# xmed-lab/MOC

Measured on AMD Instinct MI355X. Metric: meta-steps/sec (train), slides/sec (eval) on 16-shot NSCLC synthetic bags, higher is better.
Workload: dtype f32; 1 GPU; NSCLC 2-way 16-shot train loop: 32 slides/epoch x 15000 patches x 512, topj 400, topk 10, row mask on; bag_storage=fp32, arithmetic=fp32 accumulate (MFMA), parallelism=single GPU, one Adam step per slide

## Files before the change

moc_amd/csrc/moc_meta_forward.hip:

```cpp
#include <cmath>
#include <cstddef>
#include <cstdlib>
#include "moc_meta_internal.h"

int moc_check_batch(const moc_batch_t* B, const char* who);

using namespace moc_meta_internal;

namespace {

struct FwdArgs {
    const unsigned char* X;
    const int64_t* row_off;
    const int64_t* sel_row;
    const int32_t* n_sel;
    const float* cand;
    const float *W1, *b1, *W2, *b2;
    const unsigned char* W1img;
    float *H1, *gates, *mixed;
    int64_t stride;
    int64_t base_host;
    int D, C, slide0;
    uint32_t use_bits;
    int cand_mode;
// ... 245 lines not shown
        const int r = threadIdx.x >> 2, i = threadIdx.x & 3;
        float z = 0.f;
        for (int h = 0; h < H; ++h) z = fmaf(Hs[r][h], W2s[i * H + h], z);
        z += b2_pre;
        const float g = 1.f / (1.f + expf(-z));
        Gs[r][i] = g;
        if (a.gates && row0 + r < S) a.gates[(base + row0 + r) * 4 + i] = g;
    }
    __syncthreads();
    for (int e = threadIdx.x; e < 16 * C; e += 256) {
        const int r = e & 15, c = e >> 4;
        if (row0 + r >= S) continue;
        float s0 = pre_c[0], s1 = pre_c[1], s2 = pre_c[2], s3 = pre_c[3];
        if (e >= 256) {
            const float* cd = cand_row(a, base, row0 + r);
            float m1, rden;
            cand_row_norm(a, cd, m1, rden);
            cand_class_scores(a, cd, c, m1, rden, s0, s1);
            cand_row_scores(a, cd, s2, s3);
        }
        float v = 0.f;
        if (a.use_bits & 1u) v = moc_fadd(v, moc_fmul(Gs[r][0], s0));
        if (a.use_bits & 2u) v = moc_fadd(v, moc_fmul(Gs[r][1], s1));
        if (a.use_bits & 4u) v = moc_fadd(v, moc_fmul(Gs[r][2], s2));
        if (a.use_bits & 8u) v = moc_fadd(v, moc_fmul(Gs[r][3], s3));
        a.mixed[(int64_t)c * a.stride + base + row0 + r] = v;
    }
    if (TILES && a.tile_on && threadIdx.x < 16 * C) {
        const int r = threadIdx.x & 15, c = threadIdx.x >> 4;
        const bool ok = row0 + r < S;
        float v = 0.f;
        if (a.use_bits & 1u) v = moc_fadd(v, moc_fmul(Gs[r][0], pre_c[0]));
        if (a.use_bits & 2u) v = moc_fadd(v, moc_fmul(Gs[r][1], pre_c[1]));
        if (a.use_bits & 4u) v = moc_fadd(v, moc_fmul(Gs[r][2], pre_c[2]));
        if (a.use_bits & 8u) v = moc_fadd(v, moc_fmul(Gs[r][3], pre_c[3]));
        const float4 lam4 = {Gs[r][0], Gs[r][1], Gs[r][2], Gs[r][3]};
        const float4 sc4 = {pre_c[0], pre_c[1], pre_c[2], pre_c[3]};
        tile_emit(a.tile, fr.tile_slot0 / TILE_R + (int64_t)c * fr.tile_cap + blockIdx.x, ok, v, row0 + r, rid_e, lam4, sc4);
    }
    MOC_STAMP(2);
}

constexpr int FKS_PSTR = H + 4;
__host__ __device__ constexpr int fks_lds_bytes(int D) {
    return 3 * 16 * D * 2 + 4 * 16 * FKS_PSTR * 4 + 16 * (H + 1) * 4 + 16 * 4 * 4 + 4 * H * 4;
}
template <int DQ, bool STATS>
__global__ __launch_bounds__(1024) void meta_forward_ksplit_kernel(FwdArgs a) {
    extern __shared__ __attribute__((aligned(16))) unsigned char smem[];
    constexpr int D = DQ * 256;
    uint4* xt = reinterpret_cast<uint4*>(smem);
    float* part = reinterpret_cast<float*>(smem + (size_t)3 * 16 * D * 2);
    float (*Hs)[H + 1] = reinterpret_cast<float (*)[H + 1]>(part + 4 * 16 * FKS_PSTR);
    float (*Gs)[4] = reinterpret_cast<float (*)[4]>(reinterpret_cast<float*>(Hs) + 16 * (H + 1));
    float* W2s = reinterpret_cast<float*>(Gs) + 16 * 4;
    const FwdRun fr = fwd_run_setup(a);
    const int b = fr.b;
    const int64_t base = fr.base;
    const int S = fr.S >= 0 ? fr.S : a.n_sel[b];
    const int row0 = blockIdx.x * 16;
    if (row0 >= S) return;
    const int t = threadIdx.x, lane = t & 63;
    const int wave = __builtin_amdgcn_readfirstlane(t >> 6);
    const int ht = wave & 3, kq = wave >> 2;
    MOC_STAMP(0);
    MOC_STAMP_MIN(31);
    MOC_STAMP_MAX(32);
    constexpr int64_t row_bytes = (int64_t)D * 4;
    constexpr int cpl = DQ;
    const int sr = min(row0 + wave, S - 1);
    const int64_t rid = a.sel_row[base + sr];
    const unsigned char* rp = a.X + rid * row_bytes + lane * 16;
    MOC_STAMP_DRAIN(3);
    constexpr int QK = D / 128;
    const uint4* wi = reinterpret_cast<const uint4*>(fr.W1img) + ((size_t)ht * (D / 32) + (size_t)kq * QK) * 3 * 64 + lane + (rid >> 63);
    uint4 xv[cpl];
#pragma unroll
    for (int i = 0; i < cpl; ++i) xv[i] = *reinterpret_cast<const uint4*>(rp + i * 1024);
    uint4 wv[QK * 3];
#pragma unroll
    for (int q = 0; q < QK * 3; ++q) wv[q] = wi[q * 64];
    constexpr int cpr = D / 8;
    uint2* xt2 = reinterpret_cast<uint2*>(smem);
#pragma unroll
    for (int i = 0; i < cpl; ++i) {
        uint2 tv[3];
        fwd_split4(xv[i], tv);
        const int o = (wave * cpr + (((lane + i * 64) >> 1) ^ wave)) * 2 + (lane & 1);
#pragma unroll
        for (int p = 0; p < 3; ++p) xt2[p * 16 * cpr * 2 + o] = tv[p];
    }
    MOC_STAMP(5);
    __syncthreads();
    MOC_STAMP(6);
    const int C = a.C;
    float pre_c[4] = {0.f, 0.f, 0.f, 0.f};
    const int er = t & 15, ec = t >> 4;
    const bool e_ok = ec < C && row0 + er < S;
    if constexpr (STATS) {
        if (e_ok) {
            const float* cd = cand_row(a, base, row0 + er);
            float m1, rden;
            cand_row_norm(a, cd, m1, rden);
            cand_class_scores(a, cd, ec, m1, rden, pre_c[0], pre_c[1]);
            cand_row_scores(a, cd, pre_c[2], pre_c[3]);
        }
    } else {
        const float* cd = a.cand + base + min(row0 + er, S - 1);
        const int cc = ec < C ? ec : C - 1;
        pre_c[0] = cd[(int64_t)cc * a.stride];
        pre_c[1] = cd[(int64_t)(C + cc) * a.stride];
        pre_c[2] = cd[(int64_t)(2 * C) * a.stride];
        pre_c[3] = cd[(int64_t)(2 * C + 1) * a.stride];
    }
    const float w2_pre = fr.W2[t & 255];
    const float bias = fr.b1[t & 63];
    const float b2_pre = fr.b2[t & 3];
    int64_t rid_e = 0;
    if (a.tile_on) rid_e = a.sel_row[base + min(row0 + er, S - 1)];
    __builtin_amdgcn_sched_barrier(0);
    f32x4_t acc = {0.f, 0.f, 0.f, 0.f};
    {
        const int r = lane & 15;
        const uint4* xr = xt + r * cpr;
        const int c0 = kq * QK * 4 + (lane >> 4);
#pragma unroll
        for (int kk = 0; kk < QK; ++kk) {
            const int c = (c0 + kk * 4) ^ r;
            const uint4 xa[3] = {xr[c], xr[16 * cpr + c], xr[32 * cpr + c]};
            acc = fwd_mfma6(xa, wv[kk * 3], wv[kk * 3 + 1], wv[kk * 3 + 2], acc);
        }
    }
#ifdef MOC_STAMPS
    asm volatile("v_add_f32 %0, %0, 0" : "+v"(acc[0]));
#endif
    MOC_STAMP(1);
    {
        float* pp = part + (size_t)(kq * 16 + (lane >> 4) * 4) * FKS_PSTR + ht * 16 + (lane & 15);
#pragma unroll
        for (int i = 0; i < 4; ++i) pp[i * FKS_PSTR] = acc[i];
        if (t < 4 * H) W2s[t] = w2_pre;
    }
    __syncthreads();
    MOC_STAMP(7);
    {
        const int r = t >> 6, h = t & 63;
        const float* pp = part + (size_t)r * FKS_PSTR + h;
        const float pre = moc_fadd(moc_fadd(moc_fadd(pp[0], pp[16 * FKS_PSTR]), pp[32 * FKS_PSTR]), pp[48 * FKS_PSTR]);
        const float hv = fmaxf(moc_fadd(pre, bias), 0.f);
        Hs[r][h] = hv;
        if (a.H1 && row0 + r < S) a.H1[(base + row0 + r) * H + h] = hv;
    }
    __syncthreads();
    MOC_STAMP(8);
    if (t < 64) {
        const int r = t >> 2, i = t & 3;
        float z = 0.f;
        for (int h = 0; h < H; ++h) z = fmaf(Hs[r][h], W2s[i * H + h], z);
        z += b2_pre;
        const float g = 1.f / (1.f + expf(-z));
        Gs[r][i] = g;
        if (a.gates && row0 + r < S) a.gates[(base + row0 + r) * 4 + i] = g;
    }
    __syncthreads();
    MOC_STAMP(9);
    if (ec < C) {
        float v = 0.f;
        if (a.use_bits & 1u) v = moc_fadd(v, moc_fmul(Gs[er][0], pre_c[0]));
        if (a.use_bits & 2u) v = moc_fadd(v, moc_fmul(Gs[er][1], pre_c[1]));
        if (a.use_bits & 4u) v = moc_fadd(v, moc_fmul(Gs[er][2], pre_c[2]));
        if (a.use_bits & 8u) v = moc_fadd(v, moc_fmul(Gs[er][3], pre_c[3]));
        if (e_ok) a.mixed[(int64_t)ec * a.stride + base + row0 + er] = v;
        if (a.tile_on) {
            const float4 lam4 = {Gs[er][0], Gs[er][1], Gs[er][2], Gs[er][3]};
            const float4 sc4 = {pre_c[0], pre_c[1], pre_c[2], pre_c[3]};
            tile_emit(a.tile, fr.tile_slot0 / TILE_R + (int64_t)ec * fr.tile_cap + blockIdx.x, e_ok, v, row0 + er, rid_e, lam4, sc4);
        }
    }
    MOC_STAMP(2);
    MOC_STAMP_MAX(30);
}

template <bool F16>
__global__ __launch_bounds__(256) void meta_forward64_kernel(FwdArgs a) {
    __shared__ __attribute__((aligned(16))) uint4 xt[64 * 32];
    __shared__ float Hs[64][H + 1];
    __shared__ float Gs[64][4];
    __shared__ float W2s[4 * H];
    const int b = a.slide0 + blockIdx.y;
    const int64_t base = a.row_off[b];
    const int S = a.n_sel[b];
    const int row0 = blockIdx.x * 64;
    if (row0 >= S) return;
    const int lane = threadIdx.x & 63, wave = threadIdx.x >> 6;
    const int C = a.C;
    const int er = threadIdx.x & 63, ec0 = threadIdx.x >> 6;
    const bool erow_ok = row0 + er < S;
    const float* ecd = cand_row(a, base, erow_ok ? row0 + er : row0);
    float es2 = 0.f, es3 = 0.f, em1 = 0.f, erd = 0.f, es0[8], es1[8];
    if (erow_ok) {
        cand_row_scores(a, ecd, es2, es3);
        cand_row_norm(a, ecd, em1, erd);
    }
#pragma unroll
    for (int it = 0; it < 8; ++it) {
        const int c = ec0 + 4 * it;
        es0[it] = es1[it] = 0.f;
        if (erow_ok && c < C) cand_class_scores(a, ecd, c, em1, erd, es0[it], es1[it]);
    }
    const float w2_pre = a.W2[threadIdx.x & 255];
    const float bias = a.b1[wave * 16 + (lane & 15)];
    const float b2_pre = a.b2[threadIdx.x & 3];
    const int64_t row_bytes = (int64_t)a.D * 2;
    const int U = (int)(row_bytes / 512), KST = (int)(row_bytes / 64);
    const unsigned char* rp[8];
#pragma unroll
    for (int j = 0; j < 8; ++j) {
        const int sr = min(row0 + wave * 16 + 2 * j + (lane >> 5), S - 1);
        rp[j] = a.X + a.sel_row[base + sr] * row_bytes + (lane & 31) * 16;
    }
    f32x4_t acc[4];
#pragma unroll
    for (int rt = 0; rt < 4; ++rt) acc[rt] = f32x4_t{0.f, 0.f, 0.f, 0.f};
    for (int u = 0; u < U; ++u) {
        if (u > 0) __syncthreads();
        uint4 xv[8];
#pragma unroll
        for (int j = 0; j < 8; ++j) xv[j] = *reinterpret_cast<const uint4*>(rp[j] + (int64_t)u * 512);
        uint4 wv[8 * 3];
        const uint4* wi = reinterpret_cast<const uint4*>(a.W1img) + ((size_t)wave * KST + (size_t)u * 8) * 3 * 64 + lane;
#pragma unroll
        for (int q = 0; q < 8 * 3; ++q) wv[q] = wi[q * 64];
#pragma unroll
        for (int j = 0; j < 8; ++j) {
            const int r = wave * 16 + 2 * j + (lane >> 5);
            xt[r * 32 + ((lane & 31) ^ (r & 15))] = xv[j];
        }
        __syncthreads();
#pragma unroll
        for (int kk = 0; kk < 8; ++kk) {
#pragma unroll
            for (int rt = 0; rt < 4; ++rt) {
                const int r = rt * 16 + (lane & 15);
                const uint4 A = xt[r * 32 + ((kk * 4 + (lane >> 4)) ^ (r & 15))];
#pragma unroll
                for (int t = 0; t < 3; ++t) acc[rt] = moc_mfma_half<F16>(A, wv[kk * 3 + t], acc[rt]);
            }
        }
    }
    {
        const int hcol = wave * 16 + (lane & 15);
#pragma unroll
        for (int rt = 0; rt < 4; ++rt)
#pragma unroll
            for (int i = 0; i < 4; ++i) {
                const float pre = F16 ? acc[rt][i] * (1.f / MOC_F16_W1_SCALE) : acc[rt][i];
                Hs[rt * 16 + (lane >> 4) * 4 + i][hcol] = fmaxf(moc_fadd(pre, bias), 0.f);
            }
        W2s[threadIdx.x] = w2_pre;
    }
    __syncthreads();
    if (a.H1) {
        for (int e = threadIdx.x; e < 64 * H; e += 256) {
            const int r = e >> 6, h = e & 63;
            if (row0 + r < S) a.H1[(base + row0 + r) * H + h] = Hs[r][h];
        }
    }
    {
        const int r = threadIdx.x >> 2, i = threadIdx.x & 3;
        float z = 0.f;
        for (int h = 0; h < H; ++h) z = fmaf(Hs[r][h], W2s[i * H + h], z);
        z += b2_pre;
        const float g = 1.f / (1.f + expf(-z));
        Gs[r][i] = g;
        if (a.gates && row0 + r < S) a.gates[(base + row0 + r) * 4 + i] = g;
    }
    __syncthreads();
    for (int cb = 0; cb < C; cb += 32) {
        if (cb > 0) {
#pragma unroll
            for (int it = 0; it < 8; ++it) {
                const int c = cb + ec0 + 4 * it;
                if (erow_ok && c < C) cand_class_scores(a, ecd, c, em1, erd, es0[it], es1[it]);
            }
        }
#pragma unroll
        for (int it = 0; it < 8; ++it) {
            const int c = cb + ec0 + 4 * it;
            if (!erow_ok || c >= C) continue;
            float v = 0.f;
            if (a.use_bits & 1u) v = moc_fadd(v, moc_fmul(Gs[er][0], es0[it]));
            if (a.use_bits & 2u) v = moc_fadd(v, moc_fmul(Gs[er][1], es1[it]));
            if (a.use_bits & 4u) v = moc_fadd(v, moc_fmul(Gs[er][2], es2));
            if (a.use_bits & 8u) v = moc_fadd(v, moc_fmul(Gs[er][3], es3));
            a.mixed[(int64_t)c * a.stride + base + row0 + er] = v;
        }
    }
}

constexpr int F128_ROWS = 128;
constexpr int f128_kc(int st) { return st == 2 ? 2 : 1; }
constexpr int f128_wgs(int st) { return st == 2 ? 3 : 4; }
constexpr int f128_buf(int kc) { return (F128_ROWS / 16) * kc * 1024; }
constexpr int f128_xb(int kc) { return 2 * f128_buf(kc) > F128_ROWS * (H + 1) * 4 ? 2 * f128_buf(kc) : F128_ROWS * (H + 1) * 4; }
constexpr int f128_lds(int kc) { return f128_xb(kc) + F128_ROWS * 4 * 4 + 4 * H * 4; }
typedef unsigned __attribute__((ext_vector_type(4))) fu32x4_t;
template <int OFF>
__device__ __forceinline__ void fwd_lds16(fu32x4_t& dst, unsigned addr) {
    asm volatile("ds_read_b128 %0, %1 offset:%2" : "=&v"(dst) : "v"(addr), "n"(OFF) : "memory");
}
__device__ __forceinline__ void fwd_touch4(fu32x4_t (&v)[4]) {
    asm volatile("" : "+v"(v[0]), "+v"(v[1]), "+v"(v[2]), "+v"(v[3]));
}

constexpr int F128_MODELS = 4;
constexpr int F128_ENSEMBLE = 8;
constexpr int F128_BY_SLIDE = 16;
constexpr int F128_ENS_MAX_C = 64;
constexpr int f128_bound(int stm) { return (stm & F128_ENSEMBLE) ? f128_wgs(stm & 3) - 1 : f128_wgs(stm & 3); }
template <int STM, bool DENSE = false>
__global__ __launch_bounds__(256, f128_bound(STM)) void meta_forward128_kernel(FwdArgs a) {
    constexpr int ST = STM & 3;
    constexpr bool MODELS = (STM & F128_MODELS) != 0;
    constexpr bool ENS = (STM & F128_ENSEMBLE) != 0;
    constexpr bool BYS = (STM & F128_BY_SLIDE) != 0;
    static_assert(!ENS || (MODELS && DENSE), "the ensemble mode is a dense models mode");
    static_assert(!BYS || (!MODELS && !DENSE), "a model per slide: the union rows, one model each");
    constexpr int F128_KC = f128_kc(ST), F128_BUF = f128_buf(F128_KC), F128_XB = f128_xb(F128_KC);
    constexpr bool F16 = ST == 1;
    constexpr int WPC = 3 * (ST == 2 ? F128_KC / 2 : F128_KC);
    constexpr int ESZ = ST == 2 ? 4 : 2;
    extern __shared__ __attribute__((aligned(16))) unsigned char smem[];
    float (*Hs)[H + 1] = reinterpret_cast<float (*)[H + 1]>(smem);
    float (*Gs)[4] = reinterpret_cast<float (*)[4]>(smem + F128_XB);
    float* W2s = reinterpret_cast<float*>(smem + F128_XB + F128_ROWS * 4 * 4);
    const int b = a.slide0 + blockIdx.y;
    const int64_t base = a.row_off[b];
    const int S = DENSE ? (int)(a.row_off[b + 1] - base) : a.n_sel[b];
    const int row0 = blockIdx.x * F128_ROWS;
    if (row0 >= S) return;
    const int lane = threadIdx.x & 63, wave = threadIdx.x >> 6;
    const int C = a.C;
#ifdef MOC_FWD_DIAG
    const unsigned diag = a.use_bits >> 8;
#else
    constexpr unsigned diag = 0;
#endif
    const int er = threadIdx.x & 127, ec0 = threadIdx.x >> 7;
    const bool erow_ok = row0 + er < S;
    const float* ecd = DENSE ? a.stats + base + (erow_ok ? row0 + er : row0) : cand_row(a, base, erow_ok ? row0 + er : row0);
    float es2 = 0.f, es3 = 0.f, em1 = 0.f, erd = 0.f, es0[8];
    if (erow_ok) {
        cand_row_scores(a, ecd, es2, es3);
        cand_row_norm(a, ecd, em1, erd);
    }
#pragma unroll
    for (int it = 0; it < 8; ++it) {
        const int c = ec0 + 2 * it;
        es0[it] = 0.f;
        if (erow_ok && c < C) es0[it] = ecd[(int64_t)c * a.stride];
    }
    float w2_pre = a.W2[threadIdx.x & 255];
    float bias = a.b1[wave * 16 + (lane & 15)];
    float b2_pre = a.b2[threadIdx.x & 3];
    int bys_m = 0;
    if constexpr (BYS) {
        bys_m = min(max(a.model_of_slide[b], 0), a.n_runs - 1);
        const int64_t po = (int64_t)bys_m * a.par_stride;
        w2_pre = a.W2[po + (threadIdx.x & 255)];
        bias = a.b1[po + wave * 16 + (lane & 15)];
        b2_pre = a.b2[po + (threadIdx.x & 3)];
    }
    const int64_t row_bytes = (int64_t)a.D * ESZ;
    const int KK = (int)(row_bytes / 64), nchunk = KK / F128_KC;
    const unsigned char* rp[2];
    int64_t xbase = 0;
    if constexpr (DENSE) xbase = a.x_off ? a.x_off[b] : base;
#pragma unroll
    for (int j = 0; j < 2; ++j) {
        const int sr = min(row0 + (wave * 2 + j) * 16 + (lane & 15), S - 1);
        rp[j] = a.X + (DENSE ? xbase + sr : a.sel_row[base + sr]) * row_bytes + (lane >> 4) * 16;
    }
    typedef const __attribute__((address_space(1))) void* gptr_t;
    typedef __attribute__((address_space(3))) void* lptr_t;
    auto issue_x = [&](int c, int buf) {
        unsigned char* dst = smem + buf * F128_BUF;
#pragma unroll
        for (int j = 0; j < 2; ++j)
#pragma unroll
            for (int kl = 0; kl < F128_KC; ++kl)
                __builtin_amdgcn_global_load_lds((gptr_t)(rp[j] + ((int64_t)c * F128_KC + kl) * 64),
                                                 (lptr_t)(dst + ((wave * 2 + j) * F128_KC + kl) * 1024), 16, 0, 0);
    };
    int m = 0;
next_model:
    if (MODELS && m > 0) {
        const int64_t po = (int64_t)m * a.par_stride;
        const float *W2m = a.W2, *b1m = a.b1, *b2m = a.b2;
        if constexpr (ENS) asm volatile("" : "+s"(W2m), "+s"(b1m), "+s"(b2m));
        w2_pre = W2m[po + (threadIdx.x & 255)];
        bias = b1m[po + wave * 16 + (lane & 15)];
        b2_pre = b2m[po + (threadIdx.x & 3)];
    }
    int64_t cstride = a.stride;
    if constexpr (ENS) {
        asm volatile("" : "+s"(cstride), "+v"(rp[0]), "+v"(rp[1]), "+v"(ecd));
    }
    const unsigned char* w1img = MODELS ? a.W1img + (int64_t)m * a.img_stride : a.W1img;
    if constexpr (BYS) w1img += (int64_t)bys_m * a.img_stride;
    float* mixed = MODELS ? a.mixed + (int64_t)m * C * a.stride : a.mixed;
    const fu32x4_t* wimg = reinterpret_cast<const fu32x4_t*>(w1img) + (size_t)wave * (a.D / 32) * 3 * 64 + lane;
    auto load_w = [&](int c, fu32x4_t (&wv)[WPC]) {
#pragma unroll
        for (int q = 0; q < WPC; ++q) wv[q] = wimg[((size_t)c * WPC + q) * 64];
    };
    f32x4_t acc[8];
#pragma unroll
    for (int r = 0; r < 8; ++r) acc[r] = f32x4_t{0.f, 0.f, 0.f, 0.f};
    f32x4_t tot[ST == 2 ? 8 : 1] = {};
    const int qchunks = nchunk / 4;
    const unsigned lds0 = (unsigned)(uintptr_t)smem + lane * 16;
    const unsigned lds0f = (unsigned)(uintptr_t)smem + (lane >> 5) * 1024 + ((((lane >> 4) & 1) * 32) + (lane & 15)) * 16;
    auto body = [&](int c, const fu32x4_t (&cur)[WPC], fu32x4_t (&nxt)[WPC]) {
        if (c + 1 < nchunk) {
            if (!(diag & 2u)) load_w(c + 1, nxt);
            if (!(diag & 4u)) issue_x(c + 1, (c + 1) & 1);
        }
        if constexpr (ST == 2) {
            const unsigned buf = lds0f + (c & 1) * F128_BUF;
#pragma unroll
            for (int rt = 0; rt < 8; ++rt) {
                fu32x4_t P[2];
                fwd_lds16<0>(P[0], buf + rt * F128_KC * 1024);
                fwd_lds16<256>(P[1], buf + rt * F128_KC * 1024);
                asm volatile("s_waitcnt lgkmcnt(0)" ::: "memory");
                asm volatile("" : "+v"(P[0]), "+v"(P[1]));
                if (!(diag & 1u)) {
                    uint4 xa[3];
                    fwd_split8(__builtin_bit_cast(uint4, P[0]), __builtin_bit_cast(uint4, P[1]), xa);
                    acc[rt] = fwd_mfma6(xa, cur[0], cur[1], cur[2], acc[rt]);
                }
            }
            if ((c + 1) % qchunks == 0) {
                const bool first = c + 1 == qchunks;
#pragma unroll
                for (int r = 0; r < 8; ++r) fwd_fold_quarter(tot[r], acc[r], first);
            }
            __syncthreads();
            return;
        }
        const unsigned buf = lds0 + (c & 1) * F128_BUF;
        fu32x4_t A0[2], A1[2];
#pragma unroll
        for (int r = 0; r < 2; ++r) fwd_lds16<0>(A0[r], buf + (r * F128_KC + 0) * 1024);
#pragma unroll
        for (int st = 0; st < F128_KC * 4; ++st) {
            const int kl = st >> 2, g = st & 3;
            fu32x4_t (&Ac)[2] = (st & 1) ? A1 : A0;
            fu32x4_t (&An)[2] = (st & 1) ? A0 : A1;
            if (st + 1 < F128_KC * 4) {
                const int kl_n = (st + 1) >> 2, g_n = (st + 1) & 3;
#pragma unroll
                for (int r = 0; r < 2; ++r) fwd_lds16<0>(An[r], buf + ((g_n * 2 + r) * F128_KC + kl_n) * 1024);
                asm volatile("s_waitcnt lgkmcnt(2)" ::: "memory");
            } else {
                asm volatile("s_waitcnt lgkmcnt(0)" ::: "memory");
            }
            asm volatile("" : "+v"(Ac[0]), "+v"(Ac[1]));
            if (!(diag & 1u)) {
#pragma unroll
                for (int r = 0; r < 2; ++r)
#pragma unroll
                    for (int t = 0; t < 3; ++t) acc[g * 2 + r] = moc_mfma_half<F16>(Ac[r], cur[kl * 3 + t], acc[g * 2 + r]);
            }
        }
        __syncthreads();
    };
    fu32x4_t wA[WPC], wB[WPC];
    load_w(0, wA);
    issue_x(0, 0);
    __syncthreads();
    for (int c = 0; c < nchunk; c += 2) {
        body(c, wA, wB);
        if (c + 1 < nchunk) body(c + 1, wB, wA);
    }
    {
        const int hcol = wave * 16 + (lane & 15);
        if constexpr (ST == 2) {
#pragma unroll
            for (int r = 0; r < 8; ++r) acc[r] = tot[r];
        }
#pragma unroll
        for (int r = 0; r < 8; ++r)
#pragma unroll
            for (int i = 0; i < 4; ++i) {
                const float pre = F16 ? acc[r][i] * (1.f / MOC_F16_W1_SCALE) : acc[r][i];
                Hs[r * 16 + (lane >> 4) * 4 + i][hcol] = fmaxf(moc_fadd(pre, bias), 0.f);
            }
        W2s[threadIdx.x] = w2_pre;
    }
    __syncthreads();
    if (!ENS && a.H1) {
        for (int e = threadIdx.x; e < F128_ROWS * H; e += 256) {
            const int r = e >> 6, h = e & 63;
            if (row0 + r < S) a.H1[(base + row0 + r) * H + h] = Hs[r][h];
        }
    }
#pragma unroll
    for (int rr = 0; rr < 2; ++rr) {
        const int r = (threadIdx.x >> 2) + rr * 64, i = threadIdx.x & 3;
        float z = 0.f;
        for (int h = 0; h < H; ++h) z = fmaf(Hs[r][h], W2s[i * H + h], z);
        z += b2_pre;
        const float g = 1.f / (1.f + expf(-z));
        Gs[r][i] = g;
        if constexpr (ENS) {
            float* gts = a.gates;
            asm volatile("" : "+s"(gts));
            if (gts && row0 + r < S) {
                float* gp = gts + (base + row0 + r) * 4 + i;
                const float sg = m > 0 ? *gp + g : g;
                *gp = m + 1 == a.n_runs ? sg / (float)a.n_runs : sg;
            }
        } else {
            if (a.gates && row0 + r < S) a.gates[(base + row0 + r) * 4 + i] = g;
        }
    }
    __syncthreads();
    float* Ms = reinterpret_cast<float*>(smem);
    if (erow_ok && !(diag & 8u)) {
        const float g0 = Gs[er][0], g1 = Gs[er][1], g2 = Gs[er][2], g3 = Gs[er][3];
        for (int cb = 0; cb < C; cb += 16) {
            if (cb > 0 || (MODELS && m > 0 && C > 16)) {
#pragma unroll
                for (int it = 0; it < 8; ++it) {
                    const int c = cb + ec0 + 2 * it;
                    if (c < C) es0[it] = ecd[(int64_t)c * cstride];
                }
            }
            float es1[8];
#pragma unroll
            for (int it = 0; it < 8; ++it) {
                const int c = cb + ec0 + 2 * it;
                es1[it] = 0.f;
                if (c < C) es1[it] = a.cand_mode == 2 ? moc_softmax_from(es0[it], em1, erd) : ecd[(int64_t)(C + c) * cstride];
            }
#pragma unroll
            for (int it = 0; it < 8; ++it) {
                const int c = cb + ec0 + 2 * it;
                if (c >= C) continue;
                const float s1 = es1[it];
                float v = 0.f;
                if (a.use_bits & 1u) v = moc_fadd(v, moc_fmul(g0, es0[it]));
                if (a.use_bits & 2u) v = moc_fadd(v, moc_fmul(g1, s1));
                if (a.use_bits & 4u) v = moc_fadd(v, moc_fmul(g2, es2));
                if (a.use_bits & 8u) v = moc_fadd(v, moc_fmul(g3, es3));
                if constexpr (ENS) Ms[er * C + c] = v;
                else mixed[(int64_t)c * cstride + base + row0 + er] = v;
            }
        }
    }
    if constexpr (ENS) {
        __syncthreads();
        if (erow_ok) {
            const float* mr = Ms + er * C;
            const float scale = a.ens_scale;
            float mx = -INFINITY, se = 0.f;
            for (int c = 0; c < C; ++c) mx = fmaxf(mx, scale * mr[c]);
            for (int c = 0; c < C; ++c) se += expf(scale * mr[c] - mx);
            float* __restrict__ pmean = a.mixed + base + row0 + er;
            float* __restrict__ pm2 = a.H1 ? a.H1 + base + row0 + er : nullptr;
            const bool last = m + 1 == a.n_runs;
            const float kf = (float)(m + 1);
            for (int cb = 0; cb < C; cb += 16) {
                float mu[8], m2[8];
#pragma unroll
                for (int it = 0; it < 8; ++it) {
                    const int c = cb + ec0 + 2 * it;
                    mu[it] = 0.f;
                    m2[it] = 0.f;
                    if (m > 0 && c < C) {
                        mu[it] = pmean[(int64_t)c * cstride];
                        if (pm2) m2[it] = pm2[(int64_t)c * cstride];
                    }
                }
#pragma unroll
                for (int it = 0; it < 8; ++it) {
                    const int c = cb + ec0 + 2 * it;
                    if (c >= C) continue;
                    const float p = expf(scale * mr[c] - mx) / se;
                    const float d = p - mu[it];
                    const float mu1 = m > 0 ? mu[it] + d / kf : p;
                    const float m21 = m > 0 ? m2[it] + d * (p - mu1) : 0.f;
                    pmean[(int64_t)c * cstride] = mu1;
                    if (pm2) pm2[(int64_t)c * cstride] = last ? sqrtf(m21 / (float)a.n_runs) : m21;
                }
            }
        }
        __syncthreads();
    }
    if constexpr (MODELS) {
        if (++m < a.n_runs) goto next_model;
    }
}

__global__ __launch_bounds__(256) void fixed_mix_kernel(FwdArgs a, int mode) {
    const int b = a.slide0 + blockIdx.y;
    const int64_t base = a.row_off[b];
    const int S = a.n_sel[b], C = a.C;
    const int s = blockIdx.x * 256 + threadIdx.x;
    if (s >= S) return;
    const float* cd = a.cand + base + s;
    const float s2 = cd[(int64_t)(2 * C) * a.stride], s3 = cd[(int64_t)(2 * C + 1) * a.stride];
    for (int c = 0; c < C; ++c) {
        const float s0 = cd[(int64_t)c * a.stride], s1 = cd[(int64_t)(C + c) * a.stride];
        float v;
        if (mode == 0) v = moc_fadd(moc_fadd(moc_fadd(moc_fmul(0.25f, s0), moc_fmul(0.25f, s1)), moc_fmul(0.25f, s2)), moc_fmul(0.25f, s3));
        else if (mode == 1) v = moc_fadd(moc_fadd(moc_fadd(s0, s1), s2), s3);
        else v = fmaxf(fmaxf(s0, s1), fmaxf(s2, s3));
        a.mixed[(int64_t)c * a.stride + base + s] = v;
    }
}

}

namespace moc_meta_internal {

int check_meta(const moc_batch_t* B, const moc_meta_t* M, const moc_meta_ws_t* ws, const char* who,
               bool need_adam, bool need_grad, bool need_h1) {
    MOC_REQUIRE(M && ws, "%s: null meta/ws", who);
    MOC_REQUIRE(M->H == H, "%s: hidden width %d unsupported (must be %d)", who, M->H, H);
    MOC_REQUIRE(M->D == B->D, "%s: meta D=%d != batch D=%d", who, M->D, B->D);
    MOC_REQUIRE(M->W1 && M->b1 && M->W2 && M->b2, "%s: null parameter", who);
    MOC_REQUIRE((!need_h1 || (ws->H1 && ws->gates)) && ws->mixed && ws->pooled && ws->topk_idx && ws->topk_cnt && ws->loss && ws->pred,
                "%s: null work array", who);
    MOC_REQUIRE(B->sel_row && B->n_sel && B->cand, "%s: batch has no phase-A outputs", who);
    MOC_REQUIRE(!(B->flags & MOC_CAND_FROM_STATS) || !(need_adam || need_grad),
                "%s: a MOC_CAND_FROM_STATS batch has no materialised candidate scores (evaluation only)", who);
    MOC_REQUIRE(B->topk <= 256 && B->C <= 256, "%s: topk/C too large for the fused step (<= 256)", who);
    if (need_adam)
        MOC_REQUIRE(M->m_W1 && M->m_b1 && M->m_W2 && M->m_b2 && M->v_W1 && M->v_b1 && M->v_W2 && M->v_b2,
                    "%s: null Adam state", who);
    if (need_grad) MOC_REQUIRE(M->g_W1 && M->g_b1 && M->g_W2 && M->g_b2, "%s: null gradient output", who);
    if (need_adam || need_grad) MOC_REQUIRE(ws->pair_dh && ws->pair_row && ws->n_pair, "%s: null backward scratch", who);
    return MOC_OK;
}

int launch_w1_images(const moc_batch_t* B, const moc_meta_t* M, const moc_runs_t* R, hipStream_t s) {
    MOC_REQUIRE(M->W1_image, "meta: W1_image buffer is null (moc_w1_image_bytes)");
    w1_image_kernel<<<dim3(H * B->D / 256, R ? R->n_runs : 1), 256, 0, s>>>(M->W1, B->D, (unsigned char*)M->W1_image, B->dtype,
                                                                            R ? R->par_stride : 0, R ? R->image_stride : 0);
    MOC_CHECK_LAUNCH(R ? "moc_w1_image(runs)" : "moc_w1_image");
    return MOC_OK;
}

int s_bound(const moc_batch_t* B) {
    const int64_t by_sel = (int64_t)B->topj * (2 * B->C + 2);
    return (int)(by_sel < B->max_rows ? by_sel : B->max_rows);
}

}

namespace {

constexpr int F64_SINGLE_ROWS = 16384;

FwdArgs fwd_args(const moc_batch_t* B, const moc_meta_t* M, int slide0, uint32_t use_bits) {
    FwdArgs a = {};
    a.X = (const unsigned char*)B->X; a.row_off = B->row_off; a.sel_row = B->sel_row; a.n_sel = B->n_sel;
    a.cand = B->cand; a.W1 = M->W1; a.b1 = M->b1; a.W2 = M->W2; a.b2 = M->b2;
    a.W1img = (const unsigned char*)M->W1_image;
    a.stride = B->total_rows;
    a.D = B->D; a.C = B->C; a.slide0 = slide0; a.use_bits = use_bits;
    a.base_host = -1;
    a.S_host = -1;
    if (B->flags & MOC_CAND_FROM_STATS) {
        a.cand_mode = (B->flags & MOC_STATS_COMPACT) ? 2 : 1;
        a.stats = B->stats; a.sel_idx = B->sel_idx;
    }
    return a;
}

template <int MODE, bool DENSE>
int launch_f128(const FwdArgs& a, dim3 grid, int dtype, hipStream_t s, const char* who) {
    static std::once_flag attr;
    std::call_once(attr, [] {
        (void)hipFuncSetAttribute((const void*)meta_forward128_kernel<MODE + 0, DENSE>, hipFuncAttributeMaxDynamicSharedMemorySize, f128_lds(f128_kc(0)));
        (void)hipFuncSetAttribute((const void*)meta_forward128_kernel<MODE + 1, DENSE>, hipFuncAttributeMaxDynamicSharedMemorySize, f128_lds(f128_kc(1)));
        (void)hipFuncSetAttribute((const void*)meta_forward128_kernel<MODE + 2, DENSE>, hipFuncAttributeMaxDynamicSharedMemorySize, f128_lds(f128_kc(2)));
    });
    if (dtype == MOC_F16) meta_forward128_kernel<MODE + 1, DENSE><<<grid, 256, f128_lds(f128_kc(1)), s>>>(a);
    else if (dtype == MOC_BF16) meta_forward128_kernel<MODE + 0, DENSE><<<grid, 256, f128_lds(f128_kc(0)), s>>>(a);
    else meta_forward128_kernel<MODE + 2, DENSE><<<grid, 256, f128_lds(f128_kc(2)), s>>>(a);
    MOC_CHECK_LAUNCH(who);
    return MOC_OK;
}

int launch_ksplit(const FwdArgs& a, dim3 grid, hipStream_t s, const char* who) {
    static std::once_flag attr;
    std::call_once(attr, [] {
#define MOC_KS_ATTR(DQ)                                                                                                                                  \
    (void)hipFuncSetAttribute((const void*)meta_forward_ksplit_kernel<DQ, false>, hipFuncAttributeMaxDynamicSharedMemorySize, fks_lds_bytes(DQ * 256)); \
    (void)hipFuncSetAttribute((const void*)meta_forward_ksplit_kernel<DQ, true>, hipFuncAttributeMaxDynamicSharedMemorySize, fks_lds_bytes(DQ * 256))
        MOC_KS_ATTR(2); MOC_KS_ATTR(3); MOC_KS_ATTR(4);
#undef MOC_KS_ATTR
    });
    const int lds = fks_lds_bytes(a.D);
#define MOC_KS_LAUNCH(DQ)                                                                        \
    do {                                                                                         \
        if (a.cand_mode) meta_forward_ksplit_kernel<DQ, true><<<grid, 1024, lds, s>>>(a);         \
        else meta_forward_ksplit_kernel<DQ, false><<<grid, 1024, lds, s>>>(a);                    \
    } while (0)
    switch (a.D / 256) {
        case 1: MOC_KS_LAUNCH(1); break;
        case 2: MOC_KS_LAUNCH(2); break;
        case 3: MOC_KS_LAUNCH(3); break;
        default: MOC_KS_LAUNCH(4); break;
    }
#undef MOC_KS_LAUNCH
    MOC_CHECK_LAUNCH(who);
    return MOC_OK;
}

int64_t dense_rows(const moc_batch_t* B, int slide0, int n) {
    if (!B->row_off_host) return B->max_rows;
    int64_t rows = 0;
    for (int q = slide0; q < slide0 + n; ++q) {
        const int64_t nq = B->row_off_host[q + 1] - B->row_off_host[q];
        rows = nq > rows ? nq : rows;
    }
    return rows;
}

}

int moc_meta_internal::launch_forward(const moc_batch_t* B, const moc_meta_t* M, const moc_meta_ws_t* ws, int slide0, int n,
                                      uint32_t use_bits, hipStream_t s, bool emit_tiles, const moc_runs_t* runs, int64_t w2_stride) {
    MOC_REQUIRE(!(B->flags & MOC_CAND_FROM_STATS) || (B->stats && B->sel_idx),
                "moc_meta_forward: MOC_CAND_FROM_STATS needs the batch's stats and sel_idx");
    FwdArgs a = fwd_args(B, M, slide0, use_bits);
#ifdef MOC_FWD_DIAG
    if (const char* dg = getenv("MOC_FWD_DIAG")) a.use_bits |= (uint32_t)atoi(dg) << 8;
#endif
    a.H1 = ws->H1; a.gates = ws->gates; a.mixed = ws->mixed;
    if (n == 1 && B->row_off_host) a.base_host = B->row_off_host[slide0];
    if (emit_tiles) {
        MOC_REQUIRE(n == 1 && B->row_off_host && ws->tile_ws, "moc_meta_forward: tile records need one slide, row_off_host and ws->tile_ws");
        a.tile_on = 1;
        a.tile = tile_carve(ws->tile_ws, tile_slots(B->total_rows, B->n_slides, B->C));
        a.tile_cap = moc_cdiv(B->row_off_host[slide0 + 1] - a.base_host, 16);
        a.tile_slot0 = ((a.base_host >> 4) + slide0) * (int64_t)B->C * TILE_R;
    }
    dim3 grid(moc_cdiv(s_bound(B), 16), n);
    const bool s_known = n == 1 && B->n_sel_host != nullptr;
    if (s_known && !runs) {
        a.S_host = B->n_sel_host[slide0];
        MOC_REQUIRE(a.S_host >= 0 && a.S_host <= s_bound(B), "moc_meta_forward: n_sel_host[%d] = %d is not a row count of this batch (bound %d)",
                    slide0, a.S_host, s_bound(B));
        grid.x = a.S_host > 0 ? moc_cdiv(a.S_host, 16) : 1;
    }
    if (runs) {
        MOC_REQUIRE(n == 1 && a.tile_on, "moc_train_steps_runs: the batched forward needs the tile-record step");
        a.n_runs = runs->n_runs; a.slide_stride = runs->slide_stride;
        a.par_stride = runs->par_stride; a.img_stride = runs->image_stride; a.w2_stride = w2_stride;
        int s_max = 0;
        for (int r = 0; r < runs->n_runs; ++r) {
            const int sl = slide0 + r * runs->slide_stride;
            a.base_r[r] = B->row_off_host[sl];
            a.tile_cap_r[r] = moc_cdiv(B->row_off_host[sl + 1] - B->row_off_host[sl], 16);
            a.tile_slot0_r[r] = ((B->row_off_host[sl] >> 4) + sl) * (int64_t)B->C * TILE_R;
            if (s_known) {
                a.S_r[r] = B->n_sel_host[sl];
                MOC_REQUIRE(a.S_r[r] >= 0 && a.S_r[r] <= s_bound(B), "moc_train_steps_runs: n_sel_host[%d] = %d is not a row count of this batch", sl, a.S_r[r]);
                s_max = a.S_r[r] > s_max ? a.S_r[r] : s_max;
            }
        }
        if (s_known) { a.S_host = 0; grid.x = s_max > 0 ? moc_cdiv(s_max, 16) : 1; }
        grid.y = runs->n_runs;
        static const int fwd4_env = getenv("MOC_RUNS_FWD4") ? atoi(getenv("MOC_RUNS_FWD4")) : -1;
        const bool four = fwd4_env >= 0 ? fwd4_env != 0 : (int64_t)grid.x * grid.y > 512;
        if (B->dtype == MOC_F32 && four && B->C <= 16) {
            meta_forward_kernel<false, false, true><<<grid, 256, 0, s>>>(a);
            MOC_CHECK_LAUNCH("moc_meta_forward(runs, four waves)");
            return MOC_OK;
        }
        if (B->dtype == MOC_F32) {
            MOC_REQUIRE(B->D <= 1024 && B->C <= 64, "moc_train_steps_runs: fp32 bags need D <= 1024, C <= 64");
            return launch_ksplit(a, grid, s, "moc_meta_forward(runs)");
        }
        if (B->dtype == MOC_F16) meta_forward_kernel<true, true, true><<<grid, 256, 0, s>>>(a);
        else meta_forward_kernel<true, false, true><<<grid, 256, 0, s>>>(a);
        MOC_CHECK_LAUNCH("moc_meta_forward(runs)");
        return MOC_OK;
// ... 190 lines not shown
```

Baseline: 50980 meta-steps/s.

## Restructure fp32 forward chunk loop with a three-slot half-chunk ring and shared split planes

For the fp32 storage path (ST==2), each wave now streams X in half-chunks into a three-slot per-wave LDS ring, prefetching up to two halves ahead instead of double-buffering whole chunks. Each wave splits only its own rows into three planes once and writes them to a shared LDS plane area. All waves then read those planes to run the MFMA tiles, so the repeated split work and the per-tile lgkmcnt(0) stalls are removed. Weight prefetch uses raw dwordx4 loads with explicit vmcnt waits. The cost is more LDS per block (which may lower occupancy), extra barriers, and fragile hand-coded waitcnt values.

Result: no change. 50890 meta-steps/s (-0.2%).

```diff
diff --git a/moc_amd/csrc/moc_meta_forward.hip b/moc_amd/csrc/moc_meta_forward.hip
--- a/moc_amd/csrc/moc_meta_forward.hip
+++ b/moc_amd/csrc/moc_meta_forward.hip
@@ -571,7 +571,12 @@
 constexpr int f128_kc(int st) { return st == 2 ? 2 : 1; }
 constexpr int f128_wgs(int st) { return st == 2 ? 3 : 4; }
 constexpr int f128_buf(int kc) { return (F128_ROWS / 16) * kc * 1024; }
-constexpr int f128_xb(int kc) { return 2 * f128_buf(kc) > F128_ROWS * (H + 1) * 4 ? 2 * f128_buf(kc) : F128_ROWS * (H + 1) * 4; }
+constexpr int F128_RING = 3 * (F128_ROWS / 16) * 1024;
+constexpr int F128_PLANES = (F128_ROWS / 16) * 3 * 1024;
+constexpr int f128_xb(int kc) {
+    return kc == 2 ? F128_RING + F128_PLANES
+                   : 2 * f128_buf(kc) > F128_ROWS * (H + 1) * 4 ? 2 * f128_buf(kc) : F128_ROWS * (H + 1) * 4;
+}
 constexpr int f128_lds(int kc) { return f128_xb(kc) + F128_ROWS * 4 * 4 + 4 * H * 4; }
 typedef unsigned __attribute__((ext_vector_type(4))) fu32x4_t;
 template <int OFF>
@@ -596,6 +601,7 @@
     static_assert(!ENS || (MODELS && DENSE), "the ensemble mode is a dense models mode");
     static_assert(!BYS || (!MODELS && !DENSE), "a model per slide: the union rows, one model each");
     constexpr int F128_KC = f128_kc(ST), F128_BUF = f128_buf(F128_KC), F128_XB = f128_xb(F128_KC);
+    static_assert(F128_XB >= F128_ROWS * (H + 1) * 4, "Hs lies over the chunk buffers");
     constexpr bool F16 = ST == 1;
     constexpr int WPC = 3 * (ST == 2 ? F128_KC / 2 : F128_KC);
     constexpr int ESZ = ST == 2 ? 4 : 2;
@@ -661,6 +667,12 @@
                 __builtin_amdgcn_global_load_lds((gptr_t)(rp[j] + ((int64_t)c * F128_KC + kl) * 64),
                                                  (lptr_t)(dst + ((wave * 2 + j) * F128_KC + kl) * 1024), 16, 0, 0);
     };
+    auto issue_half = [&](int h) {
+        unsigned char* dst = smem + wave * (3 * 2048) + (h % 3) * 2048;
+#pragma unroll
+        for (int j = 0; j < 2; ++j)
+            __builtin_amdgcn_global_load_lds((gptr_t)(rp[j] + (int64_t)h * 64), (lptr_t)(dst + j * 1024), 16, 0, 0);
+    };
     int m = 0;
 next_model:
     if (MODELS && m > 0) {
@@ -683,40 +695,87 @@
 #pragma unroll
         for (int q = 0; q < WPC; ++q) wv[q] = wimg[((size_t)c * WPC + q) * 64];
     };
+    auto load_w_f32 = [&](int c, fu32x4_t (&wv)[WPC]) {
+        static_assert(ST != 2 || WPC == 3, "three image fragments per fp32 chunk");
+        const fu32x4_t* wp = wimg + (size_t)c * WPC * 64;
+        asm volatile("global_load_dwordx4 %0, %3, off\n\tglobal_load_dwordx4 %1, %3, off offset:1024\n\t"
+                     "global_load_dwordx4 %2, %3, off offset:2048"
+                     : "=&v"(wv[0]), "=&v"(wv[1]), "=&v"(wv[2]) : "v"(wp) : "memory");
+    };
     f32x4_t acc[8];
 #pragma unroll
     for (int r = 0; r < 8; ++r) acc[r] = f32x4_t{0.f, 0.f, 0.f, 0.f};
     f32x4_t tot[ST == 2 ? 8 : 1] = {};
     const int qchunks = nchunk / 4;
     const unsigned lds0 = (unsigned)(uintptr_t)smem + lane * 16;
-    const unsigned lds0f = (unsigned)(uintptr_t)smem + (lane >> 5) * 1024 + ((((lane >> 4) & 1) * 32) + (lane & 15)) * 16;
+    const unsigned lds0f = (unsigned)(uintptr_t)smem + wave * (3 * 2048) + ((((lane >> 4) & 1) * 32) + (lane & 15)) * 16;
     auto body = [&](int c, const fu32x4_t (&cur)[WPC], fu32x4_t (&nxt)[WPC]) {
+        if constexpr (ST == 2) {
+            if (c + 1 < nchunk) __builtin_amdgcn_s_waitcnt(0x0F72);
+            else __builtin_amdgcn_s_waitcnt(0x0F70);
+            {
+                fu32x4_t (&cw)[WPC] = const_cast<fu32x4_t (&)[WPC]>(cur);
+                asm volatile("" : "+v"(cw[0]), "+v"(cw[1]), "+v"(cw[2]) :: "memory");
+            }
+            const unsigned lbuf = lds0f + (unsigned)((2 * c + (lane >> 5)) % 3) * 2048;
+            fu32x4_t P[2][2];
+            fwd_lds16<0>(P[0][0], lbuf);
+            fwd_lds16<256>(P[0][1], lbuf);
+            fwd_lds16<1024>(P[1][0], lbuf);
+            fwd_lds16<1024 + 256>(P[1][1], lbuf);
+            asm volatile("s_waitcnt lgkmcnt(0)" ::: "memory");
+            asm volatile("" : "+v"(P[0][0]), "+v"(P[0][1]), "+v"(P[1][0]), "+v"(P[1][1]));
+            if (c + 1 < nchunk) {
+                if (!(diag & 2u)) load_w_f32(c + 1, nxt);
+                if (!(diag & 4u)) {
+                    issue_half(2 * c + 3);
+                    if (c + 2 < nchunk) issue_half(2 * c + 4);
+                }
+            }
+            uint4 xs[2][3];
+#pragma unroll
+            for (int j = 0; j < 2; ++j)
+                fwd_split8(__builtin_bit_cast(uint4, P[j][0]), __builtin_bit_cast(uint4, P[j][1]), xs[j]);
+            asm volatile("s_barrier" ::: "memory");
+            const unsigned pl = lds0 + F128_RING + wave * (2 * 3 * 1024);
+#define MOC_X(J, T) "v"(__builtin_bit_cast(fu32x4_t, xs[J][T]))
+            asm volatile("ds_write_b128 %0, %1 offset:0\n\tds_write_b128 %0, %2 offset:1024\n\tds_write_b128 %0, %3 offset:2048\n\t"
+                         "ds_write_b128 %0, %4 offset:3072\n\tds_write_b128 %0, %5 offset:4096\n\tds_write_b128 %0, %6 offset:5120\n\t"
+                         "s_waitcnt lgkmcnt(0)\n\ts_barrier"
+                         :: "v"(pl), MOC_X(0, 0), MOC_X(0, 1), MOC_X(0, 2), MOC_X(1, 0), MOC_X(1, 1), MOC_X(1, 2) : "memory");
+#undef MOC_X
+            const unsigned pbuf = lds0 + F128_RING;
+            fu32x4_t A0[3], A1[3];
+            fwd_lds16<0>(A0[0], pbuf);
+            fwd_lds16<1024>(A0[1], pbuf);
+            fwd_lds16<2048>(A0[2], pbuf);
+#define MOC_F128_TILE(RT, Ac, An)                                                                                       \
+    if ((RT) + 1 < 8) {                                                                                                 \
+        fwd_lds16<((RT) + 1) % 8 * 3072>(An[0], pbuf);                                                                  \
+        fwd_lds16<((RT) + 1) % 8 * 3072 + 1024>(An[1], pbuf);                                                           \
+        fwd_lds16<((RT) + 1) % 8 * 3072 + 2048>(An[2], pbuf);                                                           \
+        asm volatile("s_waitcnt lgkmcnt(3)" ::: "memory");                                                              \
+    } else {                                                                                                            \
+        asm volatile("s_waitcnt lgkmcnt(0)" ::: "memory");                                                              \
+    }                                                                                                                   \
+    asm volatile("" : "+v"(Ac[0]), "+v"(Ac[1]), "+v"(Ac[2]));                                                           \
+    if (!(diag & 1u)) {                                                                                                 \
+        const uint4 xa[3] = {__builtin_bit_cast(uint4, Ac[0]), __builtin_bit_cast(uint4, Ac[1]), __builtin_bit_cast(uint4, Ac[2])}; \
+        acc[RT] = fwd_mfma6(xa, cur[0], cur[1], cur[2], acc[RT]);                                                       \
+    }
+            MOC_F128_TILE(0, A0, A1) MOC_F128_TILE(1, A1, A0) MOC_F128_TILE(2, A0, A1) MOC_F128_TILE(3, A1, A0)
+            MOC_F128_TILE(4, A0, A1) MOC_F128_TILE(5, A1, A0) MOC_F128_TILE(6, A0, A1) MOC_F128_TILE(7, A1, A0)
+#undef MOC_F128_TILE
+            if ((c + 1) % qchunks == 0) {
+                const bool first = c + 1 == qchunks;
+#pragma unroll
+                for (int r = 0; r < 8; ++r) fwd_fold_quarter(tot[r], acc[r], first);
+            }
+            return;
+        }
         if (c + 1 < nchunk) {
             if (!(diag & 2u)) load_w(c + 1, nxt);
             if (!(diag & 4u)) issue_x(c + 1, (c + 1) & 1);
-        }
-        if constexpr (ST == 2) {
-            const unsigned buf = lds0f + (c & 1) * F128_BUF;
-#pragma unroll
-            for (int rt = 0; rt < 8; ++rt) {
-                fu32x4_t P[2];
-                fwd_lds16<0>(P[0], buf + rt * F128_KC * 1024);
-                fwd_lds16<256>(P[1], buf + rt * F128_KC * 1024);
-                asm volatile("s_waitcnt lgkmcnt(0)" ::: "memory");
-                asm volatile("" : "+v"(P[0]), "+v"(P[1]));
-                if (!(diag & 1u)) {
-                    uint4 xa[3];
-                    fwd_split8(__builtin_bit_cast(uint4, P[0]), __builtin_bit_cast(uint4, P[1]), xa);
-                    acc[rt] = fwd_mfma6(xa, cur[0], cur[1], cur[2], acc[rt]);
-                }
-            }
-            if ((c + 1) % qchunks == 0) {
-                const bool first = c + 1 == qchunks;
-#pragma unroll
-                for (int r = 0; r < 8; ++r) fwd_fold_quarter(tot[r], acc[r], first);
-            }
-            __syncthreads();
-            return;
         }
         const unsigned buf = lds0 + (c & 1) * F128_BUF;
         fu32x4_t A0[2], A1[2];
@@ -746,8 +805,15 @@
         __syncthreads();
     };
     fu32x4_t wA[WPC], wB[WPC];
-    load_w(0, wA);
-    issue_x(0, 0);
+    if constexpr (ST == 2) {
+        load_w_f32(0, wA);
+        issue_half(0);
+        issue_half(1);
+        if (nchunk > 1) issue_half(2);
+    } else {
+        load_w(0, wA);
+        issue_x(0, 0);
+    }
     __syncthreads();
     for (int c = 0; c < nchunk; c += 2) {
         body(c, wA, wB);
@@ -758,6 +824,7 @@
         if constexpr (ST == 2) {
 #pragma unroll
             for (int r = 0; r < 8; ++r) acc[r] = tot[r];
+            __syncthreads();
         }
 #pragma unroll
         for (int r = 0; r < 8; ++r)
```
